# yangdongchao/RSTnet

Hardware: NVIDIA H100
Metric: codec_frames_per_s (higher is better)
Workload: dtype f32

## Files before the change

rstnet_b200/csrc/gemm_tc.cu:

```cuda
#include <cstdlib>

#include "common.cuh"
#include "tc_common.cuh"
#include "../../include/rstnet_b200.h"

namespace rstnet {
extern void count_launch();
using namespace tc;

constexpr int TC_BM = 128;
constexpr int TC_BKE = 32;
constexpr int TC_A_BYTES = TC_BM * 128;
constexpr int TC_CONSUMER_WARPS = 8;
constexpr int TC_THREADS = 32 * TC_CONSUMER_WARPS + 32;
constexpr int TC_CHUNK_STAGES = 4;

struct TcParams {
  float* C;
  float* C2;
  int act2;
  long long c_i_stride, c_o_stride, c_split_stride;
  const float* R;
  long long r_i_stride, r_o_stride, r_split_stride;
  const float* bias;
  const float* scale;
  int n_split;
  int I_out, O_out, N, Kc;
  int taps, tap_di, tap_do, o_mul, kchunks;
  int pre_act, post_act, i_tiles;
  int m_tiles, n_tiles;
  int kpair;
};

template <int BN, int PREC>
struct TcCfg {
  static constexpr bool SPLIT = PREC == 0;
  static constexpr int B_BYTES = BN * 128;
  static constexpr int STAGE_BYTES = TC_A_BYTES + B_BYTES * (SPLIT ? 2 : 1);
  static constexpr int STAGES = (200 * 1024 / STAGE_BYTES) > 8 ? 8 : (200 * 1024 / STAGE_BYTES);
  static constexpr int SMEM_BYTES = STAGES * STAGE_BYTES + 1024  + 256 ;
  static constexpr int Q_PIECES = BN / 32;
  static_assert(STAGES % 2 == 0 && 2 * Q_PIECES <= STAGES, "K-pair rings and queue");
};

__device__ __forceinline__ float tf32_rna(float x) {
  const uint32_t u = __float_as_uint(x);
  return __uint_as_float((x != x ? u | 0x00400000u : u + 0x1000u) & 0xFFFFE000u);
// ... 17 lines not shown
    for (int e = 0; e < 4; ++e) {
      const uint32_t chunk = (uint32_t)(2 * k + (e >> 1));
      float v;
      asm volatile("ld.shared.f32 %0, [%1];" : "=f"(v) : "r"(st + a_row + (e & 1) * 1024u + ((chunk ^ a_sw) << 4)));
      if (PRE_ELU) {
        const float e = __expf(v) - 1.f;
        v = v > 0.f ? v : e;
      }
      if (SPLIT) {
        const bool nonfinite = !(fabsf(v) < INFINITY);
        const float h = nonfinite ? 0.f : __uint_as_float((__float_as_uint(v) + 0x1000u) & 0xFFFFE000u);
        const float d = v - h;
        ah[k][e] = __float_as_uint(h);
        al[k][e] = (__float_as_uint(d) + (nonfinite ? 0u : 0x1000u)) & 0xFFFFE000u;
      } else {
        ah[k][e] = __float_as_uint(tf32_rna(v));
      }
    }
  }
}

template <int BN, bool SPLIT>
__device__ __forceinline__ void tc_mma_stage(float (&d0)[BN / 2], float (&d1)[BN / 2], const uint32_t (&ah)[4][4],
                                             const uint32_t (&al)[4][4], uint64_t db, uint64_t dbl, bool first) {
#pragma unroll
  for (int k = 0; k < 4; ++k) {
    const uint32_t acc_in = (first && k == 0) ? 0u : 1u;
    wgmma_tf32_rs<BN>(d0, ah[k], db + (uint64_t)(2 * k), acc_in);
    if (SPLIT) {
      wgmma_tf32_rs<BN>(d1, al[k], db + (uint64_t)(2 * k), acc_in);
      wgmma_tf32_rs<BN>(d1, ah[k], dbl + (uint64_t)(2 * k), 1u);
    }
  }
}

template <int BN, int PREC, bool PRE_ELU, bool KP>
__global__ void __launch_bounds__(TC_THREADS, 1)
gemm_tc_kernel(const __grid_constant__ CUtensorMap tmA, const __grid_constant__ CUtensorMap tmW,
               const __grid_constant__ CUtensorMap tmWlo, const TcParams p) {
  using Cfg = TcCfg<BN, PREC>;
  constexpr int S = Cfg::STAGES;
  constexpr int CH = TC_CHUNK_STAGES;
  constexpr int NR = BN / 2;
  extern __shared__ uint8_t smem_raw[];
  uint8_t* smem = smem_raw + ((1024u - (smem_u32(smem_raw) & 1023u)) & 1023u);
  uint64_t* full = reinterpret_cast<uint64_t*>(smem + S * Cfg::STAGE_BYTES);
  uint64_t* empty = full + S;
  uint64_t* qfull = empty + S;
  uint64_t* qempty = qfull + 2;
  const int warp = threadIdx.x / 32, lane = threadIdx.x % 32;
  const int total_k = p.taps * p.kchunks;
  const int total_tiles = p.m_tiles * p.n_tiles;
  const int bm = KP ? TC_BM / 2 : TC_BM;
  const int R = KP ? S / 2 : S;

  if (threadIdx.x == 0) {
    for (int s = 0; s < S; ++s) {
      mbar_init(&full[s], 1);
      mbar_init(&empty[s], KP ? TC_CONSUMER_WARPS / 2 : TC_CONSUMER_WARPS);
    }
    for (int q = 0; q < 2; ++q) {
      mbar_init(&qfull[q], 128);
      mbar_init(&qempty[q], 128);
    }
    fence_barrier_init();
  }
  __syncthreads();

  if (warp == TC_CONSUMER_WARPS) {
    if (elect_one()) {
      tma_prefetch_desc(&tmA);
      tma_prefetch_desc(&tmW);
      if (Cfg::SPLIT) tma_prefetch_desc(&tmWlo);
      int pos0 = 0, ph0 = 0, pos1 = 0, ph1 = 0;
      for (int t = blockIdx.x; t < total_tiles; t += gridDim.x) {
        const int nt = t % p.n_tiles, mt = t / p.n_tiles;
        const int i0 = (mt % p.i_tiles) * bm, ot = mt / p.i_tiles, n0 = nt * BN;
        for (int kit = 0; kit < total_k; ++kit) {
          const int w = KP ? (kit / TC_CHUNK_STAGES) & 1 : 0;
          const int pos = w ? pos1 : pos0, ph = w ? ph1 : ph0;
          const int s = w * R + pos;
          const int npos = pos + 1 == R ? 0 : pos + 1, nph = ph ^ (npos == 0);
          if (w) { pos1 = npos; ph1 = nph; } else { pos0 = npos; ph0 = nph; }
          mbar_wait(&empty[s], ph ^ 1);
          const int tap = kit / p.kchunks, kc = kit % p.kchunks;
          uint8_t* st = smem + s * Cfg::STAGE_BYTES;
          mbar_arrive_expect_tx(&full[s], Cfg::STAGE_BYTES - (TC_BM - bm) * 128);
          tma_load_3d(st, &tmA, &full[s], kc * TC_BKE, i0 + tap * p.tap_di, ot * p.o_mul + tap * p.tap_do);
          tma_load_2d(st + TC_A_BYTES, &tmW, &full[s], kit * TC_BKE, n0);
          if (Cfg::SPLIT) tma_load_2d(st + TC_A_BYTES + Cfg::B_BYTES, &tmWlo, &full[s], kit * TC_BKE, n0);
        }
      }
    }
    return;
  }

  const int wg = warp / 4, wq = warp % 4, gq = lane / 4, tq = lane % 4;
  const int r0 = (KP ? 0 : wg * 64) + wq * 16 + gq;
  const uint32_t a_row = (uint32_t)r0 * 128u + (uint32_t)tq * 4u, a_sw = (uint32_t)(r0 & 7);
  const uint32_t smem0 = smem_u32(smem);
  float acc[NR], d0[NR], d1[NR];
#pragma unroll
  for (int j = 0; j < NR; ++j) d0[j] = d1[j] = 0.f;
  const int nch = (total_k + CH - 1) / CH;
  const bool sender = KP && wg == 1;
  auto qel = [&](int q, int j) {
    return reinterpret_cast<float*>(smem + (q * Cfg::Q_PIECES + j / 16) * Cfg::STAGE_BYTES + TC_A_BYTES / 2) +
           (j % 16) * 128 + (threadIdx.x & 127);
  };
  int qn = 0;
  auto take_queued = [&]() {
    mbar_wait(&qfull[qn & 1], (qn >> 1) & 1);
#pragma unroll
    for (int j = 0; j < NR; ++j) acc[j] += *qel(qn & 1, j);
    mbar_arrive(&qempty[qn & 1]);
    ++qn;
  };
  const int base = KP ? wg * R : 0;
  int pos = 0, ph = 0;
  for (int t = blockIdx.x; t < total_tiles; t += gridDim.x) {
    const int nt = t % p.n_tiles, mt = t / p.n_tiles;
    const int i0 = (mt % p.i_tiles) * bm, ot = mt / p.i_tiles, n0 = nt * BN;
#pragma unroll
    for (int j = 0; j < NR; ++j) acc[j] = 0.f;
    for (int c = KP ? wg : 0; c < nch; c += KP ? 2 : 1) {
      const int k0 = c * CH;
      const int nst = total_k - k0 < CH ? total_k - k0 : CH;
      for (int u = 0; u < nst; ++u) {
        const int s = base + pos;
        mbar_wait(&full[s], ph);
        const uint32_t st = smem0 + (uint32_t)(s * Cfg::STAGE_BYTES);
        uint32_t ah[4][4], al[4][4];
        tc_build_a<Cfg::SPLIT, PRE_ELU>(st, a_row, a_sw, ah, al);
        const uint64_t db = gmma_desc_sw128(st + TC_A_BYTES);
        const uint64_t dbl = gmma_desc_sw128(st + TC_A_BYTES + Cfg::B_BYTES);
        wgmma_fence();
        tc_mma_stage<BN, Cfg::SPLIT>(d0, d1, ah, al, db, dbl, u == 0);
        wgmma_commit();
        wgmma_wait<0>();
        __syncwarp();
        if (lane == 0) mbar_arrive(&empty[s]);
        pos = pos + 1 == R ? 0 : pos + 1;
        ph ^= pos == 0;
      }
      fence_acc(d0);
      if (Cfg::SPLIT) fence_acc(d1);
      if (sender) {
        mbar_wait(&qempty[qn & 1], ((qn >> 1) & 1) ^ 1);
#pragma unroll
        for (int j = 0; j < NR; ++j) *qel(qn & 1, j) = Cfg::SPLIT ? d0[j] + d1[j] : d0[j];
        mbar_arrive(&qfull[qn & 1]);
        ++qn;
      } else {
        if (KP && c > 0) take_queued();
#pragma unroll
        for (int j = 0; j < NR; ++j) acc[j] += Cfg::SPLIT ? d0[j] + d1[j] : d0[j];
      }
    }
    if (KP && !sender && nch % 2 == 0) take_queued();
    if (sender) continue;
#pragma unroll
    for (int h = 0; h < 2; ++h) {
      const int i = i0 + r0 + 8 * h;
      if (i >= p.I_out) continue;
      float* crow = p.C + (long long)ot * p.c_o_stride + (long long)i * p.c_i_stride;
      float* crow2 = p.C2 ? p.C2 + (long long)ot * p.c_o_stride + (long long)i * p.c_i_stride : nullptr;
      const float* rrow = p.R ? p.R + (long long)ot * p.r_o_stride + (long long)i * p.r_i_stride : nullptr;
#pragma unroll
      for (int b = 0; b < BN / 8; ++b) {
        const int n = n0 + 8 * b + 2 * tq;
        if (n < p.N) {
          float2 v = make_float2(acc[4 * b + 2 * h], acc[4 * b + 2 * h + 1]);
          if (p.bias) {
            const float2 bb = *reinterpret_cast<const float2*>(p.bias + n);
            v.x += bb.x; v.y += bb.y;
          }
          if (p.scale) {
            const float2 ss = *reinterpret_cast<const float2*>(p.scale + n);
            v.x *= ss.x; v.y *= ss.y;
          }
          long long coff = n, roff = n;
          if (p.n_split > 0) {
            const int j = n / p.n_split, co = n % p.n_split;
            coff = (long long)j * p.c_split_stride + co;
            roff = (long long)j * p.r_split_stride + co;
          }
          if (rrow) {
            const float2 rr = *reinterpret_cast<const float2*>(rrow + roff);
            v.x += rr.x; v.y += rr.y;
          }
          if (crow2)
            *reinterpret_cast<float2*>(crow2 + coff) = make_float2(act_tc(v.x, p.act2), act_tc(v.y, p.act2));
          *reinterpret_cast<float2*>(crow + coff) = make_float2(act_tc(v.x, p.post_act), act_tc(v.y, p.post_act));
        }
      }
    }
  }
}

constexpr int RB_B_BYTES = 64 * 128;
constexpr int RB_STAGE_BYTES = TC_A_BYTES + 2 * RB_B_BYTES;
constexpr int RB_STAGES = 6;

struct RbParams {
  float* out;
  long long o_i_stride, o_o_stride;
  const float* b1;
  const float* b2;
  int I_out, i_tiles, m_tiles;
};

template <int C>
struct RbCfg {
  static constexpr int N1 = C / 2;
  static constexpr int KCH = C / 32;
  static constexpr int P1 = 3 * KCH;
  static constexpr int NS = C / 64;
  static constexpr int K2 = N1 / 32;
  static constexpr int H_BYTES = K2 * TC_A_BYTES;
  static constexpr int SMEM_BYTES = RB_STAGES * RB_STAGE_BYTES + H_BYTES + 1024  + 256 ;
  static constexpr bool ring_ok() {
    for (int j = 0; j < NS; ++j)
      for (int kc = 0; kc < KCH; ++kc)
        if ((P1 + j) % RB_STAGES == (2 * KCH + kc) % RB_STAGES) return false;
    return RB_STAGES >= KCH + NS;
  }
  static_assert(ring_ok(), "ring too small for the held residual stages");
  static_assert(K2 * 2 * RB_B_BYTES <= RB_STAGE_BYTES, "a phase-2 slice must fit one stage");
};

template <int C>
__global__ void __launch_bounds__(TC_THREADS, 1)
resblock_tc_kernel(const __grid_constant__ CUtensorMap tmY, const __grid_constant__ CUtensorMap tmW1,
                   const __grid_constant__ CUtensorMap tmW1lo, const __grid_constant__ CUtensorMap tmW2,
                   const __grid_constant__ CUtensorMap tmW2lo, const RbParams p) {
  using Cfg = RbCfg<C>;
  constexpr int S = RB_STAGES;
  constexpr int CH = TC_CHUNK_STAGES;
  constexpr int N1 = Cfg::N1, NR1 = N1 / 2, KCH = Cfg::KCH, P1 = Cfg::P1;
  extern __shared__ uint8_t smem_raw[];
  uint8_t* smem = smem_raw + ((1024u - (smem_u32(smem_raw) & 1023u)) & 1023u);
  uint8_t* hs = smem + S * RB_STAGE_BYTES;
  uint64_t* full = reinterpret_cast<uint64_t*>(hs + Cfg::H_BYTES);
  uint64_t* empty = full + S;
  const int warp = threadIdx.x / 32, lane = threadIdx.x % 32;

  if (threadIdx.x == 0) {
    for (int s = 0; s < S; ++s) {
      mbar_init(&full[s], 1);
      mbar_init(&empty[s], TC_CONSUMER_WARPS);
    }
    fence_barrier_init();
  }
  __syncthreads();

  if (warp == TC_CONSUMER_WARPS) {
    if (elect_one()) {
      tma_prefetch_desc(&tmY);
      tma_prefetch_desc(&tmW1);
      tma_prefetch_desc(&tmW1lo);
      tma_prefetch_desc(&tmW2);
      tma_prefetch_desc(&tmW2lo);
      int g = 0;
      for (int t = blockIdx.x; t < p.m_tiles; t += gridDim.x) {
        const int i0 = (t % p.i_tiles) * TC_BM, ot = t / p.i_tiles;
        for (int kit = 0; kit < P1; ++kit, ++g) {
          const int s = g % S;
          mbar_wait(&empty[s], ((g / S) & 1) ^ 1);
          const int tap = kit / KCH, kc = kit % KCH;
          uint8_t* st = smem + s * RB_STAGE_BYTES;
          mbar_arrive_expect_tx(&full[s], TC_A_BYTES + 2 * N1 * 128);
          tma_load_3d(st, &tmY, &full[s], kc * TC_BKE, i0, ot + tap);
          tma_load_2d(st + TC_A_BYTES, &tmW1, &full[s], kit * TC_BKE, 0);
          tma_load_2d(st + TC_A_BYTES + RB_B_BYTES, &tmW1lo, &full[s], kit * TC_BKE, 0);
        }
        for (int ns = 0; ns < Cfg::NS; ++ns, ++g) {
          const int s = g % S;
          mbar_wait(&empty[s], ((g / S) & 1) ^ 1);
          uint8_t* st = smem + s * RB_STAGE_BYTES;
          mbar_arrive_expect_tx(&full[s], Cfg::K2 * 2 * RB_B_BYTES);
#pragma unroll
          for (int kc = 0; kc < Cfg::K2; ++kc) {
            tma_load_2d(st + kc * 2 * RB_B_BYTES, &tmW2, &full[s], kc * TC_BKE, ns * 64);
            tma_load_2d(st + kc * 2 * RB_B_BYTES + RB_B_BYTES, &tmW2lo, &full[s], kc * TC_BKE, ns * 64);
          }
        }
      }
    }
    return;
  }

  const int wg = warp / 4, wq = warp % 4, gq = lane / 4, tq = lane % 4;
  const int r0 = wg * 64 + wq * 16 + gq;
  const uint32_t a_row = (uint32_t)r0 * 128u + (uint32_t)tq * 4u, a_sw = (uint32_t)(r0 & 7);
  const uint32_t smem0 = smem_u32(smem), hs0 = smem_u32(hs);
  int g = 0;
  for (int t = blockIdx.x; t < p.m_tiles; t += gridDim.x) {
    const int i0 = (t % p.i_tiles) * TC_BM, ot = t / p.i_tiles;
    const int g_res = g + 2 * KCH;
    {
      float acc[NR1], d0[NR1], d1[NR1];
#pragma unroll
      for (int j = 0; j < NR1; ++j) acc[j] = d0[j] = d1[j] = 0.f;
      for (int k0 = 0; k0 < P1; k0 += CH) {
        const int nst = P1 - k0 < CH ? P1 - k0 : CH;
        for (int u = 0; u < nst; ++u, ++g) {
          const int s = g % S;
          mbar_wait(&full[s], (g / S) & 1);
          const uint32_t st = smem0 + (uint32_t)(s * RB_STAGE_BYTES);
          uint32_t ah[4][4], al[4][4];
          tc_build_a<true, true>(st, a_row, a_sw, ah, al);
          wgmma_fence();
          tc_mma_stage<N1, true>(d0, d1, ah, al, gmma_desc_sw128(st + TC_A_BYTES), gmma_desc_sw128(st + TC_A_BYTES + RB_B_BYTES),
                                 u == 0);
          wgmma_commit();
          wgmma_wait<0>();
          __syncwarp();
          if (lane == 0 && k0 + u < 2 * KCH) mbar_arrive(&empty[s]);
        }
        fence_acc(d0);
        fence_acc(d1);
#pragma unroll
        for (int j = 0; j < NR1; ++j) acc[j] += d0[j] + d1[j];
      }
      named_bar_sync(1 + wg, 128);
#pragma unroll
      for (int hh = 0; hh < 2; ++hh) {
        const int r = r0 + 8 * hh;
#pragma unroll
        for (int b = 0; b < N1 / 8; ++b) {
          const int n = 8 * b + 2 * tq;
          const float2 bb = *reinterpret_cast<const float2*>(p.b1 + n);
          float2 v = make_float2(acc[4 * b + 2 * hh], acc[4 * b + 2 * hh + 1]);
          v.x += bb.x; v.y += bb.y;
          const uint32_t cc = (uint32_t)(n % 32);
          const uint32_t addr = hs0 + (uint32_t)(n / 32) * TC_A_BYTES + (uint32_t)r * 128u + (((cc >> 2) ^ (uint32_t)(r & 7)) << 4) +
                                (cc & 3u) * 4u;
          asm volatile("st.shared.v2.f32 [%0], {%1, %2};" ::"r"(addr), "f"(act_tc(v.x, ACT_ELU)), "f"(act_tc(v.y, ACT_ELU))
                       : "memory");
        }
      }
      named_bar_sync(1 + wg, 128);
    }
    for (int ns = 0; ns < Cfg::NS; ++ns, ++g) {
      const int s = g % S;
      mbar_wait(&full[s], (g / S) & 1);
      const uint32_t st = smem0 + (uint32_t)(s * RB_STAGE_BYTES);
      float acc[32], d0[32], d1[32];
#pragma unroll
      for (int j = 0; j < 32; ++j) d0[j] = d1[j] = 0.f;
#pragma unroll
      for (int kc = 0; kc < Cfg::K2; ++kc) {
        uint32_t ah[4][4], al[4][4];
        tc_build_a<true, false>(hs0 + (uint32_t)(kc * TC_A_BYTES), a_row, a_sw, ah, al);
        const uint32_t wst = st + (uint32_t)(kc * 2 * RB_B_BYTES);
        wgmma_fence();
        tc_mma_stage<64, true>(d0, d1, ah, al, gmma_desc_sw128(wst), gmma_desc_sw128(wst + RB_B_BYTES), kc == 0);
        wgmma_commit();
        wgmma_wait<0>();
      }
      __syncwarp();
      if (lane == 0) mbar_arrive(&empty[s]);
      fence_acc(d0);
      fence_acc(d1);
#pragma unroll
      for (int j = 0; j < 32; ++j) {
        acc[j] = 0.f;
        acc[j] += d0[j] + d1[j];
      }
#pragma unroll
      for (int hh = 0; hh < 2; ++hh) {
        const int r = r0 + 8 * hh;
        const int i = i0 + r;
        if (i >= p.I_out) continue;
        float* orow = p.out + (long long)ot * p.o_o_stride + (long long)i * p.o_i_stride;
#pragma unroll
        for (int b = 0; b < 8; ++b) {
          const int n = ns * 64 + 8 * b + 2 * tq;
          const float2 bb = *reinterpret_cast<const float2*>(p.b2 + n);
          float2 v = make_float2(acc[4 * b + 2 * hh], acc[4 * b + 2 * hh + 1]);
          v.x += bb.x; v.y += bb.y;
          const uint32_t cc = (uint32_t)(n % 32);
          const int rs = (g_res + n / 32) % S;
          const float2 rr = *reinterpret_cast<const float2*>(smem + rs * RB_STAGE_BYTES + r * 128 +
                                                             (((cc >> 2) ^ (uint32_t)(r & 7)) << 4) + (cc & 3u) * 4u);
          v.x += rr.x; v.y += rr.y;
          *reinterpret_cast<float2*>(orow + n) = make_float2(act_tc(v.x, ACT_ELU), act_tc(v.y, ACT_ELU));
        }
      }
      __syncwarp();
      if (lane == 0) {
        mbar_arrive(&empty[(g_res + 2 * ns) % S]);
        mbar_arrive(&empty[(g_res + 2 * ns + 1) % S]);
      }
    }
  }
}

typedef CUresult (*EncodeTiledFn)(CUtensorMap*, CUtensorMapDataType, cuuint32_t, void*, const cuuint64_t*, const cuuint64_t*,
                                  const cuuint32_t*, const cuuint32_t*, CUtensorMapInterleave, CUtensorMapSwizzle,
                                  CUtensorMapL2promotion, CUtensorMapFloatOOBfill);

static EncodeTiledFn get_encode_fn() {
  static EncodeTiledFn fn = nullptr;
  if (!fn) {
    void* p = nullptr;
    cudaDriverEntryPointQueryResult q;
    if (cudaGetDriverEntryPoint("cuTensorMapEncodeTiled", &p, cudaEnableDefault, &q) == cudaSuccess && p) fn = (EncodeTiledFn)p;
  }
  return fn;
}

}
using namespace rstnet;

struct rstnet_tc_plan {
  CUtensorMap tmA, tmW, tmWlo;
  TcParams p;
  dim3 grid;
  int bn, prec;
};

template <int BN, int PREC, bool PRE_ELU, bool KP>
static int tc_launch(const rstnet_tc_plan* pl, cudaStream_t st) {
  using Cfg = TcCfg<BN, PREC>;
  static unsigned long long attr = 0;
  smem_optin(gemm_tc_kernel<BN, PREC, PRE_ELU, KP>, Cfg::SMEM_BYTES, attr);
  gemm_tc_kernel<BN, PREC, PRE_ELU, KP><<<pl->grid, TC_THREADS, Cfg::SMEM_BYTES, st>>>(pl->tmA, pl->tmW, pl->tmWlo, pl->p);
// ... 126 lines not shown
  RSTNET_REQUIRE(d->Y && d->W1 && d->W1_lo && d->b1 && d->W2 && d->W2_lo && d->b2 && d->out, "tc_resblock_create: null pointer");
  const int Cc = d->channels;
  RSTNET_REQUIRE(Cc == 64 || Cc == 128, "tc_resblock_create: channels must be 64 or 128 (got %d)", Cc);
  RSTNET_REQUIRE(d->I_out > 0 && d->O_out > 0 && d->y_rows >= d->O_out + 2, "tc_resblock_create: bad shape");
  RSTNET_REQUIRE((uintptr_t)d->Y % 16 == 0 && (uintptr_t)d->W1 % 16 == 0 && (uintptr_t)d->W1_lo % 16 == 0 && (uintptr_t)d->W2 % 16 == 0 &&
                     (uintptr_t)d->W2_lo % 16 == 0 && (uintptr_t)d->out % 16 == 0 && (uintptr_t)d->b1 % 8 == 0 &&
                     (uintptr_t)d->b2 % 8 == 0 && d->y_i_stride % 4 == 0 && d->y_o_stride % 4 == 0 && d->out_i_stride % 4 == 0 &&
                     d->out_o_stride % 4 == 0,
                 "tc_resblock_create: 16-byte alignment required");
  RSTNET_REQUIRE(get_encode_fn() != nullptr, "tc_resblock_create: cuTensorMapEncodeTiled unavailable (no CUDA driver?)");
  rstnet_tc_resblock_plan* pl = new rstnet_tc_resblock_plan();
  pl->channels = Cc;
  int r;
  {
    cuuint64_t gdim[3] = {(cuuint64_t)Cc, (cuuint64_t)d->I_out, (cuuint64_t)d->y_rows};
    cuuint64_t gstr[2] = {(cuuint64_t)d->y_i_stride * 4, (cuuint64_t)d->y_o_stride * 4};
    cuuint32_t box[3] = {TC_BKE, TC_BM, 1};
    cuuint32_t estr[3] = {1, 1, 1};
    r = (int)get_encode_fn()(&pl->tmY, CU_TENSOR_MAP_DATA_TYPE_FLOAT32, 3, (void*)d->Y, gdim, gstr, box, estr, CU_TENSOR_MAP_INTERLEAVE_NONE,
                             CU_TENSOR_MAP_SWIZZLE_128B, CU_TENSOR_MAP_L2_PROMOTION_L2_128B, CU_TENSOR_MAP_FLOAT_OOB_FILL_NONE);
  }
  if (r == CUDA_SUCCESS) r = encode_2d(&pl->tmW1, d->W1, 3 * Cc, Cc / 2, Cc / 2);
  if (r == CUDA_SUCCESS) r = encode_2d(&pl->tmW1lo, d->W1_lo, 3 * Cc, Cc / 2, Cc / 2);
  if (r == CUDA_SUCCESS) r = encode_2d(&pl->tmW2, d->W2, Cc / 2, Cc, 64);
  if (r == CUDA_SUCCESS) r = encode_2d(&pl->tmW2lo, d->W2_lo, Cc / 2, Cc, 64);
  if (r != CUDA_SUCCESS) {
    delete pl;
    set_error("tc_resblock_create: cuTensorMapEncodeTiled failed with %d", r);
    return 3;
  }
  RbParams& p = pl->p;
  p.out = d->out; p.o_i_stride = d->out_i_stride; p.o_o_stride = d->out_o_stride;
  p.b1 = d->b1; p.b2 = d->b2;
  p.I_out = d->I_out;
  p.i_tiles = ceil_div(d->I_out, TC_BM);
  p.m_tiles = p.i_tiles * d->O_out;
  const int sms = sm_count();
  pl->grid = dim3((unsigned)(p.m_tiles < sms ? p.m_tiles : sms));
  *out = pl;
  return 0;
}

template <int Cc>
static int rb_launch(const rstnet_tc_resblock_plan* pl, cudaStream_t st) {
  constexpr int smem = RbCfg<Cc>::SMEM_BYTES;
  static unsigned long long attr = 0;
  smem_optin(resblock_tc_kernel<Cc>, smem, attr);
  resblock_tc_kernel<Cc><<<pl->grid, TC_THREADS, smem, st>>>(pl->tmY, pl->tmW1, pl->tmW1lo, pl->tmW2, pl->tmW2lo, pl->p);
  count_launch();
  return check_launch("tc_resblock");
}

extern "C" int rstnet_tc_resblock_run(const rstnet_tc_resblock_plan* pl, rstnet_stream_t stream) {
  RSTNET_REQUIRE(pl != nullptr, "tc_resblock_run: null plan");
  cudaStream_t st = (cudaStream_t)stream;
  return pl->channels == 64 ? rb_launch<64>(pl, st) : rb_launch<128>(pl, st);
}

extern "C" void rstnet_tc_resblock_destroy(rstnet_tc_resblock_plan* pl) { delete pl; }
extern "C" int rstnet_tc_gemm_grid(const rstnet_tc_plan* pl, int32_t* gx, int32_t* gy, int32_t* bn) {
  if (!pl) return 1;
  *gx = ceil_div(pl->p.I_out, TC_BM) * pl->p.O_out; *gy = pl->p.n_tiles; *bn = pl->bn;
  return 0;
}
extern "C" int rstnet_tc_gemm_kpair(const rstnet_tc_plan* pl, int32_t* on) {
  if (!pl) return 1;
  *on = pl->p.kpair;
  return 0;
}

namespace rstnet {
__global__ void tf32_split_kernel(const float* __restrict__ x, float* __restrict__ hi, float* __restrict__ lo, long long n) {
  for (long long i = (long long)blockIdx.x * blockDim.x + threadIdx.x; i < n; i += (long long)gridDim.x * blockDim.x) {
    const float v = x[i], h = tf32_rna(v);
    hi[i] = h;
    lo[i] = tf32_rna_lo(v, h);
  }
}
}

extern "C" int rstnet_tf32_split_f32(const float* x, float* hi, float* lo, int64_t n, rstnet_stream_t stream) {
// ... 9 lines not shown
```

rstnet_b200/csrc/tc_common.cuh:

```cuda
#pragma once
#include <cuda.h>
#include <cuda_runtime.h>
#include <cstdint>

namespace rstnet {
namespace tc {

__device__ __forceinline__ uint32_t smem_u32(const void* p) { return static_cast<uint32_t>(__cvta_generic_to_shared(p)); }

__device__ __forceinline__ bool elect_one() {
  uint32_t pred = 0;
  asm volatile(
      "{\n\t.reg .b32 rx;\n\t.reg .pred px;\n\t"
      "elect.sync rx|px, 0xFFFFFFFF;\n\t"
      "selp.u32 %0, 1, 0, px;\n\t}"
      : "=r"(pred));
  return pred != 0;
}

__device__ __forceinline__ void mbar_init(uint64_t* bar, uint32_t count) {
  asm volatile("mbarrier.init.shared::cta.b64 [%0], %1;" ::"r"(smem_u32(bar)), "r"(count));
}
__device__ __forceinline__ void fence_barrier_init() { asm volatile("fence.mbarrier_init.release.cluster;" ::: "memory"); }
__device__ __forceinline__ void mbar_arrive(uint64_t* bar) {
// ... 5 lines not shown
}
__device__ __forceinline__ bool mbar_try_wait(uint64_t* bar, uint32_t parity) {
  uint32_t ok;
  asm volatile(
      "{\n\t.reg .pred p;\n\t"
      "mbarrier.try_wait.parity.shared::cta.b64 p, [%1], %2;\n\t"
      "selp.u32 %0, 1, 0, p;\n\t}"
      : "=r"(ok)
      : "r"(smem_u32(bar)), "r"(parity)
      : "memory");
  return ok != 0;
}
__device__ __forceinline__ void mbar_wait(uint64_t* bar, uint32_t parity) {
  while (!mbar_try_wait(bar, parity)) {
  }
}

__device__ __forceinline__ void tma_prefetch_desc(const CUtensorMap* m) {
  asm volatile("prefetch.tensormap [%0];" ::"l"(reinterpret_cast<uint64_t>(m)) : "memory");
}
__device__ __forceinline__ void tma_load_2d(void* dst, const CUtensorMap* m, uint64_t* bar, int c0, int c1) {
  asm volatile("cp.async.bulk.tensor.2d.shared::cta.global.mbarrier::complete_tx::bytes [%0], [%1, {%3, %4}], [%2];" ::"r"(
                   smem_u32(dst)),
               "l"(reinterpret_cast<uint64_t>(m)), "r"(smem_u32(bar)), "r"(c0), "r"(c1)
               : "memory");
}
__device__ __forceinline__ void tma_load_3d(void* dst, const CUtensorMap* m, uint64_t* bar, int c0, int c1, int c2) {
  asm volatile("cp.async.bulk.tensor.3d.shared::cta.global.mbarrier::complete_tx::bytes [%0], [%1, {%3, %4, %5}], [%2];" ::"r"(
                   smem_u32(dst)),
               "l"(reinterpret_cast<uint64_t>(m)), "r"(smem_u32(bar)), "r"(c0), "r"(c1), "r"(c2)
               : "memory");
}
__device__ __forceinline__ void named_bar_sync(int id, int nthreads) { asm volatile("bar.sync %0, %1;" ::"r"(id), "r"(nthreads) : "memory"); }

__device__ __forceinline__ uint64_t gmma_desc_sw128(uint32_t saddr) {
  uint64_t d = 0;
  d |= (uint64_t)((saddr & 0x3FFFF) >> 4);
  d |= (uint64_t)1 << 16;
  d |= (uint64_t)(1024 >> 4) << 32;
  d |= (uint64_t)1 << 62;
  return d;
}
__device__ __forceinline__ void wgmma_fence() { asm volatile("wgmma.fence.sync.aligned;" ::: "memory"); }
__device__ __forceinline__ void wgmma_commit() { asm volatile("wgmma.commit_group.sync.aligned;" ::: "memory"); }
template <int N>
__device__ __forceinline__ void wgmma_wait() { asm volatile("wgmma.wait_group.sync.aligned %0;" ::"n"(N) : "memory"); }
template <int NR>
__device__ __forceinline__ void fence_acc(float (&d)[NR]) {
#pragma unroll
  for (int i = 0; i < NR; ++i) asm volatile("" : "+f"(d[i])::"memory");
}

__device__ __forceinline__ void wgmma_tf32_rs_n32(float (&d)[16], const uint32_t (&a)[4], uint64_t bdesc, uint32_t scale_d) {
  asm volatile(
      "{\n\t.reg .pred p;\n\tsetp.ne.b32 p, %21, 0;\n\t"
      "wgmma.mma_async.sync.aligned.m64n32k8.f32.tf32.tf32 "
      "{%0, %1, %2, %3, %4, %5, %6, %7, %8, %9, %10, %11, %12, %13, %14, %15}, "
      "{%16, %17, %18, %19}, %20, p, 1, 1;\n\t}"
      : "+f"(d[0]), "+f"(d[1]), "+f"(d[2]), "+f"(d[3]), "+f"(d[4]), "+f"(d[5]), "+f"(d[6]), "+f"(d[7]), "+f"(d[8]), "+f"(d[9]), "+f"(d[10]), "+f"(d[11]), "+f"(d[12]), "+f"(d[13]), "+f"(d[14]), "+f"(d[15])
      : "r"(a[0]), "r"(a[1]), "r"(a[2]), "r"(a[3]), "l"(bdesc), "r"(scale_d));
}

__device__ __forceinline__ void wgmma_tf32_rs_n64(float (&d)[32], const uint32_t (&a)[4], uint64_t bdesc, uint32_t scale_d) {
  asm volatile(
      "{\n\t.reg .pred p;\n\tsetp.ne.b32 p, %37, 0;\n\t"
      "wgmma.mma_async.sync.aligned.m64n64k8.f32.tf32.tf32 "
// ... 73 lines not shown
```

rstnet_b200/ops.py:

```python
from __future__ import annotations

import ctypes as C
import gc
from typing import Optional

import torch

from . import _lib
from ._lib import ACT_ELU, ACT_GELU, ACT_NONE, GemmRowsArgs, RowCopy, TcGemmDesc


def _stream() -> int:
    return torch.cuda.current_stream().cuda_stream


def capture(fn) -> torch.cuda.CUDAGraph:
    g = torch.cuda.CUDAGraph()
    enabled = gc.isenabled()
    gc.disable()
    try:
        with torch.cuda.graph(g):
            fn()
    finally:
        if enabled:
# ... 78 lines not shown
    def run(self):
        _lib.check(_lib.lib().rstnet_tc_gemm_run(self._h, _stream()), "tc_gemm_run")

    def __del__(self):
        h = getattr(self, "_h", None)
        if h:
            try:
                _lib.lib().rstnet_tc_gemm_destroy(h)
            except Exception:
                pass
            self._h = None


class TcResblock:

    def __init__(self, Y, y_off, y_i_stride, y_o_stride, y_rows, I_out, O_out, W1, W1_lo, b1, W2, W2_lo, b2, out, out_off,
                 out_i_stride, out_o_stride):
        _cuda(Y, W1, W1_lo, b1, W2, W2_lo, b2, out)
        Cc = W2.shape[0]
        assert tuple(W1.shape) == (Cc // 2, 3 * Cc) and tuple(W2.shape) == (Cc, Cc // 2), (W1.shape, W2.shape)
        d = _lib.TcResblockDesc()
        d.Y = Y.data_ptr() + 4 * y_off
        d.y_i_stride, d.y_o_stride = y_i_stride, y_o_stride
        d.channels, d.I_out, d.O_out, d.y_rows = Cc, I_out, O_out, y_rows
        d.W1, d.W1_lo, d.b1 = W1.data_ptr(), W1_lo.data_ptr(), b1.data_ptr()
        d.W2, d.W2_lo, d.b2 = W2.data_ptr(), W2_lo.data_ptr(), b2.data_ptr()
        d.out = out.data_ptr() + 4 * out_off
        d.out_i_stride, d.out_o_stride = out_i_stride, out_o_stride
        self._keep = (Y, W1, W1_lo, b1, W2, W2_lo, b2, out)
        self.shape = dict(C=Cc, I=I_out, O=O_out)
        n = I_out * O_out
        self.flops = 2.0 * n * (W1.numel() + W2.numel())
        self.bytes = 4.0 * (Cc * I_out * (O_out + 2) + 2 * (W1.numel() + W2.numel()) + b1.numel() + b2.numel() + n * Cc)
        self._h = C.c_void_p()
        _lib.check(_lib.lib().rstnet_tc_resblock_create(C.byref(d), C.byref(self._h)), "tc_resblock_create")

    def run(self):
        _lib.check(_lib.lib().rstnet_tc_resblock_run(self._h, _stream()), "tc_resblock_run")

    def __del__(self):
        h = getattr(self, "_h", None)
        if h:
            try:
                _lib.lib().rstnet_tc_resblock_destroy(h)
            except Exception:
                pass
            self._h = None


def conv1d_cin1(x, x_bs, x_ts, w, bias, out, out_off, out_bs, out_ts, batch, T, Cout, k, post_act=ACT_NONE, out2=None,
                out2_off=0, act2=ACT_NONE):
    _cuda(x, w, out, out2)
    _lib.check(_lib.lib().rstnet_conv1d_cin1_f32(x.data_ptr(), x_bs, x_ts, w.data_ptr(), _p(bias), out.data_ptr() + 4 * out_off,
                                                 None if out2 is None else out2.data_ptr() + 4 * out2_off, out_bs, out_ts,
                                                 batch, T, Cout, k, post_act, act2, _stream()), "conv1d_cin1")


def conv1d_cout1(x, x_bs, x_ts, w, bias, out, out_bs, batch, T, Cin, k):
    _cuda(x, w, out)
    _lib.check(_lib.lib().rstnet_conv1d_cout1_f32(x.data_ptr(), x_bs, x_ts, w.data_ptr(), _p(bias), out.data_ptr(), out_bs,
                                                  batch, T, Cin, k, _stream()), "conv1d_cout1")


def convtr1d_depthwise(x, x_bs, x_ts, w, out, out_off, out_bs, out_ts, batch, T, Cch, stride):
    _cuda(x, w, out)
    _lib.check(_lib.lib().rstnet_convtr1d_depthwise_f32(x.data_ptr(), x_bs, x_ts, w.data_ptr(), out.data_ptr() + 4 * out_off,
# ... 114 lines not shown
```

Baseline: 44550.

## Overlap consecutive WGMMA stages and add warpgroup register reallocation

Consumers now double-buffer A fragments and issue the next stage's WGMMA before waiting on the previous one (wait_group 1), releasing smem stages one step later. The producer becomes a full warpgroup that lowers its register budget via setmaxnreg while consumers raise theirs, and in KP mode two producer warps each feed their own half of the stages. The resblock second GEMM also batches all K2 MMAs before a single wait. This is meant to hide A-fragment construction and WGMMA latency behind each other. In exchange it raises register pressure from the doubled fragment arrays and adds more complex barrier release ordering.

New measurement: 45390, median of 6. 1.02x the previous value.

```diff
diff --git a/rstnet_b200/csrc/gemm_tc.cu b/rstnet_b200/csrc/gemm_tc.cu
--- a/rstnet_b200/csrc/gemm_tc.cu
+++ b/rstnet_b200/csrc/gemm_tc.cu
@@ -12,7 +12,9 @@
 constexpr int TC_BKE = 32;
 constexpr int TC_A_BYTES = TC_BM * 128;
 constexpr int TC_CONSUMER_WARPS = 8;
-constexpr int TC_THREADS = 32 * TC_CONSUMER_WARPS + 32;
+constexpr int TC_THREADS = 32 * TC_CONSUMER_WARPS + 128;
+constexpr int TC_PRODUCER_REGS = 40;
+constexpr int TC_CONSUMER_REGS = 232;
 constexpr int TC_CHUNK_STAGES = 4;
 
 struct TcParams {
@@ -96,6 +98,37 @@
       wgmma_tf32_rs<BN>(d1, ah[k], dbl + (uint64_t)(2 * k), 1u);
     }
   }
+}
+
+template <int BN, bool SPLIT, bool PRE_ELU, class Take, class Addr, class Release>
+__device__ __forceinline__ void tc_chunk(float (&d0)[BN / 2], float (&d1)[BN / 2], int nst, uint32_t a_row, uint32_t a_sw,
+                                         uint32_t b_lo, Take take, Addr addr, Release release) {
+  uint32_t ah0[4][4], al0[4][4], ah1[4][4], al1[4][4];
+  auto issue = [&](uint32_t (&ah)[4][4], uint32_t (&al)[4][4], bool first) {
+    const int tk = take();
+    const uint32_t st = addr(tk);
+    tc_build_a<SPLIT, PRE_ELU>(st, a_row, a_sw, ah, al);
+    wgmma_fence();
+    tc_mma_stage<BN, SPLIT>(d0, d1, ah, al, gmma_desc_sw128(st + TC_A_BYTES), gmma_desc_sw128(st + b_lo), first);
+    wgmma_commit();
+    return tk;
+  };
+  int held = -1, u = 0;
+  for (; u + 2 <= nst; u += 2) {
+    const int t0 = issue(ah0, al0, u == 0);
+    wgmma_wait<1>();
+    if (held >= 0) release(held);
+    held = issue(ah1, al1, false);
+    wgmma_wait<1>();
+    release(t0);
+  }
+  int tail = -1;
+  if (u < nst) tail = issue(ah0, al0, u == 0);
+  wgmma_wait<0>();
+  if (held >= 0) release(held);
+  if (tail >= 0) release(tail);
+  fence_acc(d0);
+  if (SPLIT) fence_acc(d1);
 }
 
 template <int BN, int PREC, bool PRE_ELU, bool KP>
@@ -131,34 +164,39 @@
   }
   __syncthreads();
 
-  if (warp == TC_CONSUMER_WARPS) {
-    if (elect_one()) {
+  if (warp >= TC_CONSUMER_WARPS) {
+    setmaxnreg_dec<TC_PRODUCER_REGS>();
+    const int w = warp - TC_CONSUMER_WARPS;
+    if (w < (KP ? 2 : 1) && elect_one()) {
       tma_prefetch_desc(&tmA);
       tma_prefetch_desc(&tmW);
       if (Cfg::SPLIT) tma_prefetch_desc(&tmWlo);
-      int pos0 = 0, ph0 = 0, pos1 = 0, ph1 = 0;
+      int pos = 0, ph = 0;
+      const int nch = (total_k + TC_CHUNK_STAGES - 1) / TC_CHUNK_STAGES;
       for (int t = blockIdx.x; t < total_tiles; t += gridDim.x) {
         const int nt = t % p.n_tiles, mt = t / p.n_tiles;
         const int i0 = (mt % p.i_tiles) * bm, ot = mt / p.i_tiles, n0 = nt * BN;
-        for (int kit = 0; kit < total_k; ++kit) {
-          const int w = KP ? (kit / TC_CHUNK_STAGES) & 1 : 0;
-          const int pos = w ? pos1 : pos0, ph = w ? ph1 : ph0;
-          const int s = w * R + pos;
-          const int npos = pos + 1 == R ? 0 : pos + 1, nph = ph ^ (npos == 0);
-          if (w) { pos1 = npos; ph1 = nph; } else { pos0 = npos; ph0 = nph; }
-          mbar_wait(&empty[s], ph ^ 1);
-          const int tap = kit / p.kchunks, kc = kit % p.kchunks;
-          uint8_t* st = smem + s * Cfg::STAGE_BYTES;
-          mbar_arrive_expect_tx(&full[s], Cfg::STAGE_BYTES - (TC_BM - bm) * 128);
-          tma_load_3d(st, &tmA, &full[s], kc * TC_BKE, i0 + tap * p.tap_di, ot * p.o_mul + tap * p.tap_do);
-          tma_load_2d(st + TC_A_BYTES, &tmW, &full[s], kit * TC_BKE, n0);
-          if (Cfg::SPLIT) tma_load_2d(st + TC_A_BYTES + Cfg::B_BYTES, &tmWlo, &full[s], kit * TC_BKE, n0);
+        for (int c = w; c < nch; c += KP ? 2 : 1) {
+          const int kend = (c + 1) * TC_CHUNK_STAGES < total_k ? (c + 1) * TC_CHUNK_STAGES : total_k;
+          for (int kit = c * TC_CHUNK_STAGES; kit < kend; ++kit) {
+            const int s = w * R + pos;
+            mbar_wait(&empty[s], ph ^ 1);
+            pos = pos + 1 == R ? 0 : pos + 1;
+            ph ^= pos == 0;
+            const int tap = kit / p.kchunks, kc = kit % p.kchunks;
+            uint8_t* st = smem + s * Cfg::STAGE_BYTES;
+            mbar_arrive_expect_tx(&full[s], Cfg::STAGE_BYTES - (TC_BM - bm) * 128);
+            tma_load_3d(st, &tmA, &full[s], kc * TC_BKE, i0 + tap * p.tap_di, ot * p.o_mul + tap * p.tap_do);
+            tma_load_2d(st + TC_A_BYTES, &tmW, &full[s], kit * TC_BKE, n0);
+            if (Cfg::SPLIT) tma_load_2d(st + TC_A_BYTES + Cfg::B_BYTES, &tmWlo, &full[s], kit * TC_BKE, n0);
+          }
         }
       }
     }
     return;
   }
 
+  setmaxnreg_inc<TC_CONSUMER_REGS>();
   const int wg = warp / 4, wq = warp % 4, gq = lane / 4, tq = lane % 4;
   const int r0 = (KP ? 0 : wg * 64) + wq * 16 + gq;
   const uint32_t a_row = (uint32_t)r0 * 128u + (uint32_t)tq * 4u, a_sw = (uint32_t)(r0 & 7);
@@ -182,6 +220,18 @@
   };
   const int base = KP ? wg * R : 0;
   int pos = 0, ph = 0;
+  auto take = [&]() {
+    const int s = base + pos;
+    mbar_wait(&full[s], ph);
+    pos = pos + 1 == R ? 0 : pos + 1;
+    ph ^= pos == 0;
+    return s;
+  };
+  auto addr = [&](int s) { return smem0 + (uint32_t)(s * Cfg::STAGE_BYTES); };
+  auto release = [&](int s) {
+    __syncwarp();
+    if (lane == 0) mbar_arrive(&empty[s]);
+  };
   for (int t = blockIdx.x; t < total_tiles; t += gridDim.x) {
     const int nt = t % p.n_tiles, mt = t / p.n_tiles;
     const int i0 = (mt % p.i_tiles) * bm, ot = mt / p.i_tiles, n0 = nt * BN;
@@ -190,25 +240,7 @@
     for (int c = KP ? wg : 0; c < nch; c += KP ? 2 : 1) {
       const int k0 = c * CH;
       const int nst = total_k - k0 < CH ? total_k - k0 : CH;
-      for (int u = 0; u < nst; ++u) {
-        const int s = base + pos;
-        mbar_wait(&full[s], ph);
-        const uint32_t st = smem0 + (uint32_t)(s * Cfg::STAGE_BYTES);
-        uint32_t ah[4][4], al[4][4];
-        tc_build_a<Cfg::SPLIT, PRE_ELU>(st, a_row, a_sw, ah, al);
-        const uint64_t db = gmma_desc_sw128(st + TC_A_BYTES);
-        const uint64_t dbl = gmma_desc_sw128(st + TC_A_BYTES + Cfg::B_BYTES);
-        wgmma_fence();
-        tc_mma_stage<BN, Cfg::SPLIT>(d0, d1, ah, al, db, dbl, u == 0);
-        wgmma_commit();
-        wgmma_wait<0>();
-        __syncwarp();
-        if (lane == 0) mbar_arrive(&empty[s]);
-        pos = pos + 1 == R ? 0 : pos + 1;
-        ph ^= pos == 0;
-      }
-      fence_acc(d0);
-      if (Cfg::SPLIT) fence_acc(d1);
+      tc_chunk<BN, Cfg::SPLIT, PRE_ELU>(d0, d1, nst, a_row, a_sw, TC_A_BYTES + Cfg::B_BYTES, take, addr, release);
       if (sender) {
         mbar_wait(&qempty[qn & 1], ((qn >> 1) & 1) ^ 1);
 #pragma unroll
@@ -318,8 +350,9 @@
   }
   __syncthreads();
 
-  if (warp == TC_CONSUMER_WARPS) {
-    if (elect_one()) {
+  if (warp >= TC_CONSUMER_WARPS) {
+    setmaxnreg_dec<TC_PRODUCER_REGS>();
+    if (warp == TC_CONSUMER_WARPS && elect_one()) {
       tma_prefetch_desc(&tmY);
       tma_prefetch_desc(&tmW1);
       tma_prefetch_desc(&tmW1lo);
@@ -354,36 +387,31 @@
     return;
   }
 
+  setmaxnreg_inc<TC_CONSUMER_REGS>();
   const int wg = warp / 4, wq = warp % 4, gq = lane / 4, tq = lane % 4;
   const int r0 = wg * 64 + wq * 16 + gq;
   const uint32_t a_row = (uint32_t)r0 * 128u + (uint32_t)tq * 4u, a_sw = (uint32_t)(r0 & 7);
   const uint32_t smem0 = smem_u32(smem), hs0 = smem_u32(hs);
   int g = 0;
+  auto take = [&]() {
+    mbar_wait(&full[g % S], (g / S) & 1);
+    return g++;
+  };
+  auto addr = [&](int gi) { return smem0 + (uint32_t)((gi % S) * RB_STAGE_BYTES); };
   for (int t = blockIdx.x; t < p.m_tiles; t += gridDim.x) {
     const int i0 = (t % p.i_tiles) * TC_BM, ot = t / p.i_tiles;
     const int g_res = g + 2 * KCH;
+    auto release = [&](int gi) {
+      __syncwarp();
+      if (lane == 0 && gi < g_res) mbar_arrive(&empty[gi % S]);
+    };
     {
       float acc[NR1], d0[NR1], d1[NR1];
 #pragma unroll
       for (int j = 0; j < NR1; ++j) acc[j] = d0[j] = d1[j] = 0.f;
       for (int k0 = 0; k0 < P1; k0 += CH) {
         const int nst = P1 - k0 < CH ? P1 - k0 : CH;
-        for (int u = 0; u < nst; ++u, ++g) {
-          const int s = g % S;
-          mbar_wait(&full[s], (g / S) & 1);
-          const uint32_t st = smem0 + (uint32_t)(s * RB_STAGE_BYTES);
-          uint32_t ah[4][4], al[4][4];
-          tc_build_a<true, true>(st, a_row, a_sw, ah, al);
-          wgmma_fence();
-          tc_mma_stage<N1, true>(d0, d1, ah, al, gmma_desc_sw128(st + TC_A_BYTES), gmma_desc_sw128(st + TC_A_BYTES + RB_B_BYTES),
-                                 u == 0);
-          wgmma_commit();
-          wgmma_wait<0>();
-          __syncwarp();
-          if (lane == 0 && k0 + u < 2 * KCH) mbar_arrive(&empty[s]);
-        }
-        fence_acc(d0);
-        fence_acc(d1);
+        tc_chunk<N1, true, true>(d0, d1, nst, a_row, a_sw, TC_A_BYTES + RB_B_BYTES, take, addr, release);
 #pragma unroll
         for (int j = 0; j < NR1; ++j) acc[j] += d0[j] + d1[j];
       }
@@ -413,16 +441,16 @@
       float acc[32], d0[32], d1[32];
 #pragma unroll
       for (int j = 0; j < 32; ++j) d0[j] = d1[j] = 0.f;
+      uint32_t ah[Cfg::K2][4][4], al[Cfg::K2][4][4];
 #pragma unroll
       for (int kc = 0; kc < Cfg::K2; ++kc) {
-        uint32_t ah[4][4], al[4][4];
-        tc_build_a<true, false>(hs0 + (uint32_t)(kc * TC_A_BYTES), a_row, a_sw, ah, al);
+        tc_build_a<true, false>(hs0 + (uint32_t)(kc * TC_A_BYTES), a_row, a_sw, ah[kc], al[kc]);
         const uint32_t wst = st + (uint32_t)(kc * 2 * RB_B_BYTES);
         wgmma_fence();
-        tc_mma_stage<64, true>(d0, d1, ah, al, gmma_desc_sw128(wst), gmma_desc_sw128(wst + RB_B_BYTES), kc == 0);
+        tc_mma_stage<64, true>(d0, d1, ah[kc], al[kc], gmma_desc_sw128(wst), gmma_desc_sw128(wst + RB_B_BYTES), kc == 0);
         wgmma_commit();
-        wgmma_wait<0>();
-      }
+      }
+      wgmma_wait<0>();
       __syncwarp();
       if (lane == 0) mbar_arrive(&empty[s]);
       fence_acc(d0);
diff --git a/rstnet_b200/csrc/tc_common.cuh b/rstnet_b200/csrc/tc_common.cuh
--- a/rstnet_b200/csrc/tc_common.cuh
+++ b/rstnet_b200/csrc/tc_common.cuh
@@ -61,6 +61,11 @@
                : "memory");
 }
 __device__ __forceinline__ void named_bar_sync(int id, int nthreads) { asm volatile("bar.sync %0, %1;" ::"r"(id), "r"(nthreads) : "memory"); }
+
+template <int N>
+__device__ __forceinline__ void setmaxnreg_dec() { asm volatile("setmaxnreg.dec.sync.aligned.u32 %0;" ::"n"(N)); }
+template <int N>
+__device__ __forceinline__ void setmaxnreg_inc() { asm volatile("setmaxnreg.inc.sync.aligned.u32 %0;" ::"n"(N)); }
 
 __device__ __forceinline__ uint64_t gmma_desc_sw128(uint32_t saddr) {
   uint64_t d = 0;
```

## Add window-walking resblock kernel for 64 channels with resident weights and row reuse

Applied to the files above, without the earlier changes.

Adds a new persistent resblock kernel for C=64. Each CTA walks a contiguous run of output rows and keeps a 4-slot ring of input rows, so the three conv taps reuse rows already in shared memory instead of reloading three per tile. W1 and W2 (hi/lo) are loaded once per CTA and stay resident rather than being streamed per tile. The Python side adds an L2 byte-count estimate. This cuts redundant global/L2 traffic, at the cost of serializing the wgmma waits per stage and possibly unbalanced run boundaries.

Result: no change. 44760 before, 44830 after, median of 6 (+0.2%).

```diff
diff --git a/rstnet_b200/csrc/gemm_tc.cu b/rstnet_b200/csrc/gemm_tc.cu
--- a/rstnet_b200/csrc/gemm_tc.cu
+++ b/rstnet_b200/csrc/gemm_tc.cu
@@ -271,7 +271,7 @@
   long long o_i_stride, o_o_stride;
   const float* b1;
   const float* b2;
-  int I_out, i_tiles, m_tiles;
+  int I_out, O_out, i_tiles, m_tiles;
 };
 
 template <int C>
@@ -458,6 +458,198 @@
         mbar_arrive(&empty[(g_res + 2 * ns + 1) % S]);
       }
     }
+  }
+}
+
+namespace rbw {
+constexpr int C = 64, N1 = 32, KCH = 2, P1 = 3 * KCH;
+constexpr int ROW_BYTES = KCH * TC_A_BYTES;
+constexpr int SLOTS = 4;
+constexpr int W1_STAGE = N1 * 128;
+constexpr int W2_BYTES = C * 128;
+constexpr int WIN = 0;
+constexpr int W1HI = WIN + SLOTS * ROW_BYTES;
+constexpr int W1LO = W1HI + P1 * W1_STAGE;
+constexpr int W2HI = W1LO + P1 * W1_STAGE;
+constexpr int W2LO = W2HI + W2_BYTES;
+constexpr int HS = W2LO + W2_BYTES;
+constexpr int BARS = HS + TC_A_BYTES;
+constexpr int W_BYTES = 2 * P1 * W1_STAGE + 2 * W2_BYTES;
+constexpr int SMEM_BYTES = BARS + 1024  + 256 ;
+static_assert(SMEM_BYTES <= 227 * 1024, "window, weights and h must fit one SM");
+
+struct Run {
+  int it, o0, o1;
+};
+__device__ __forceinline__ Run run_at(long long q, long long q_end, int O_out) {
+  Run r;
+  r.it = (int)(q / O_out);
+  r.o0 = (int)(q % O_out);
+  const long long left = q_end - q;
+  r.o1 = left < (long long)(O_out - r.o0) ? r.o0 + (int)left : O_out;
+  return r;
+}
+}
+
+__global__ void __launch_bounds__(TC_THREADS, 1)
+resblock_walk_kernel(const __grid_constant__ CUtensorMap tmY, const __grid_constant__ CUtensorMap tmW1,
+                     const __grid_constant__ CUtensorMap tmW1lo, const __grid_constant__ CUtensorMap tmW2,
+                     const __grid_constant__ CUtensorMap tmW2lo, const RbParams p) {
+  using namespace rbw;
+  constexpr int CH = TC_CHUNK_STAGES;
+  constexpr int NR1 = N1 / 2;
+  extern __shared__ uint8_t smem_raw[];
+  uint8_t* smem = smem_raw + ((1024u - (smem_u32(smem_raw) & 1023u)) & 1023u);
+  uint64_t* full = reinterpret_cast<uint64_t*>(smem + BARS);
+  uint64_t* empty = full + SLOTS;
+  uint64_t* wfull = empty + SLOTS;
+  const int warp = threadIdx.x / 32, lane = threadIdx.x % 32;
+  const long long items = (long long)p.m_tiles;
+  const long long q_begin = items * blockIdx.x / gridDim.x, q_end = items * (blockIdx.x + 1) / gridDim.x;
+
+  if (threadIdx.x == 0) {
+    for (int s = 0; s < SLOTS; ++s) {
+      mbar_init(&full[s], 1);
+      mbar_init(&empty[s], TC_CONSUMER_WARPS);
+    }
+    mbar_init(wfull, 1);
+    fence_barrier_init();
+  }
+  __syncthreads();
+
+  if (warp == TC_CONSUMER_WARPS) {
+    if (elect_one()) {
+      tma_prefetch_desc(&tmY);
+      tma_prefetch_desc(&tmW1);
+      tma_prefetch_desc(&tmW1lo);
+      tma_prefetch_desc(&tmW2);
+      tma_prefetch_desc(&tmW2lo);
+      mbar_arrive_expect_tx(wfull, W_BYTES);
+      for (int kit = 0; kit < P1; ++kit) {
+        tma_load_2d(smem + W1HI + kit * W1_STAGE, &tmW1, wfull, kit * TC_BKE, 0);
+        tma_load_2d(smem + W1LO + kit * W1_STAGE, &tmW1lo, wfull, kit * TC_BKE, 0);
+      }
+      tma_load_2d(smem + W2HI, &tmW2, wfull, 0, 0);
+      tma_load_2d(smem + W2LO, &tmW2lo, wfull, 0, 0);
+      int g = 0;
+      for (long long q = q_begin; q < q_end;) {
+        const Run r = run_at(q, q_end, p.O_out);
+        q += r.o1 - r.o0;
+        for (int row = r.o0; row < r.o1 + 2; ++row, ++g) {
+          const int s = g % SLOTS;
+          mbar_wait(&empty[s], ((g / SLOTS) & 1) ^ 1);
+          uint8_t* st = smem + WIN + s * ROW_BYTES;
+          mbar_arrive_expect_tx(&full[s], ROW_BYTES);
+#pragma unroll
+          for (int kc = 0; kc < KCH; ++kc) tma_load_3d(st + kc * TC_A_BYTES, &tmY, &full[s], kc * TC_BKE, r.it * TC_BM, row);
+        }
+      }
+    }
+    return;
+  }
+
+  const int wg = warp / 4, wq = warp % 4, gq = lane / 4, tq = lane % 4;
+  const int r0 = wg * 64 + wq * 16 + gq;
+  const uint32_t a_row = (uint32_t)r0 * 128u + (uint32_t)tq * 4u, a_sw = (uint32_t)(r0 & 7);
+  const uint32_t smem0 = smem_u32(smem), hs0 = smem0 + HS;
+  mbar_wait(wfull, 0);
+  int g = 0;
+  for (long long q = q_begin; q < q_end;) {
+    const Run run = run_at(q, q_end, p.O_out);
+    q += run.o1 - run.o0;
+    const int i0 = run.it * TC_BM;
+    for (int ot = run.o0; ot < run.o1; ++ot) {
+      const int g0 = g + (ot - run.o0);
+      {
+        float acc[NR1], d0[NR1], d1[NR1];
+#pragma unroll
+        for (int j = 0; j < NR1; ++j) acc[j] = d0[j] = d1[j] = 0.f;
+        for (int k0 = 0; k0 < P1; k0 += CH) {
+          const int nst = P1 - k0 < CH ? P1 - k0 : CH;
+          for (int u = 0; u < nst; ++u) {
+            const int kit = k0 + u, tap = kit / KCH, kc = kit % KCH;
+            const int gr = g0 + tap, s = gr % SLOTS;
+            mbar_wait(&full[s], (gr / SLOTS) & 1);
+            const uint32_t st = smem0 + (uint32_t)(WIN + s * ROW_BYTES + kc * TC_A_BYTES);
+            uint32_t ah[4][4], al[4][4];
+            tc_build_a<true, true>(st, a_row, a_sw, ah, al);
+            wgmma_fence();
+            tc_mma_stage<N1, true>(d0, d1, ah, al, gmma_desc_sw128(smem0 + W1HI + kit * W1_STAGE),
+                                   gmma_desc_sw128(smem0 + W1LO + kit * W1_STAGE), u == 0);
+            wgmma_commit();
+            wgmma_wait<0>();
+            __syncwarp();
+            if (lane == 0 && kit == KCH - 1) mbar_arrive(&empty[s]);
+          }
+          fence_acc(d0);
+          fence_acc(d1);
+#pragma unroll
+          for (int j = 0; j < NR1; ++j) acc[j] += d0[j] + d1[j];
+        }
+        named_bar_sync(1 + wg, 128);
+#pragma unroll
+        for (int hh = 0; hh < 2; ++hh) {
+          const int r = r0 + 8 * hh;
+#pragma unroll
+          for (int b = 0; b < N1 / 8; ++b) {
+            const int n = 8 * b + 2 * tq;
+            const float2 bb = *reinterpret_cast<const float2*>(p.b1 + n);
+            float2 v = make_float2(acc[4 * b + 2 * hh], acc[4 * b + 2 * hh + 1]);
+            v.x += bb.x; v.y += bb.y;
+            const uint32_t cc = (uint32_t)(n % 32);
+            const uint32_t addr = hs0 + (uint32_t)r * 128u + (((cc >> 2) ^ (uint32_t)(r & 7)) << 4) + (cc & 3u) * 4u;
+            asm volatile("st.shared.v2.f32 [%0], {%1, %2};" ::"r"(addr), "f"(act_tc(v.x, ACT_ELU)), "f"(act_tc(v.y, ACT_ELU))
+                         : "memory");
+          }
+        }
+        named_bar_sync(1 + wg, 128);
+      }
+      float acc[32], d0[32], d1[32];
+#pragma unroll
+      for (int j = 0; j < 32; ++j) d0[j] = d1[j] = 0.f;
+      {
+        uint32_t ah[4][4], al[4][4];
+        tc_build_a<true, false>(hs0, a_row, a_sw, ah, al);
+        wgmma_fence();
+        tc_mma_stage<64, true>(d0, d1, ah, al, gmma_desc_sw128(smem0 + W2HI), gmma_desc_sw128(smem0 + W2LO), true);
+        wgmma_commit();
+        wgmma_wait<0>();
+      }
+      fence_acc(d0);
+      fence_acc(d1);
+#pragma unroll
+      for (int j = 0; j < 32; ++j) {
+        acc[j] = 0.f;
+        acc[j] += d0[j] + d1[j];
+      }
+      const uint8_t* yres = smem + WIN + ((g0 + 2) % SLOTS) * ROW_BYTES;
+#pragma unroll
+      for (int hh = 0; hh < 2; ++hh) {
+        const int r = r0 + 8 * hh;
+        const int i = i0 + r;
+        if (i >= p.I_out) continue;
+        float* orow = p.out + (long long)ot * p.o_o_stride + (long long)i * p.o_i_stride;
+#pragma unroll
+        for (int b = 0; b < 8; ++b) {
+          const int n = 8 * b + 2 * tq;
+          const float2 bb = *reinterpret_cast<const float2*>(p.b2 + n);
+          float2 v = make_float2(acc[4 * b + 2 * hh], acc[4 * b + 2 * hh + 1]);
+          v.x += bb.x; v.y += bb.y;
+          const uint32_t cc = (uint32_t)(n % 32);
+          const float2 rr = *reinterpret_cast<const float2*>(yres + (n / 32) * TC_A_BYTES + r * 128 +
+                                                             (((cc >> 2) ^ (uint32_t)(r & 7)) << 4) + (cc & 3u) * 4u);
+          v.x += rr.x; v.y += rr.y;
+          *reinterpret_cast<float2*>(orow + n) = make_float2(act_tc(v.x, ACT_ELU), act_tc(v.y, ACT_ELU));
+        }
+      }
+    }
+    const int n_out = run.o1 - run.o0;
+    __syncwarp();
+    if (lane == 0) {
+      mbar_arrive(&empty[(g + n_out) % SLOTS]);
+      mbar_arrive(&empty[(g + n_out + 1) % SLOTS]);
+    }
+    g += n_out + 2;
   }
 }
 
@@ -650,7 +842,7 @@
   RbParams& p = pl->p;
   p.out = d->out; p.o_i_stride = d->out_i_stride; p.o_o_stride = d->out_o_stride;
   p.b1 = d->b1; p.b2 = d->b2;
-  p.I_out = d->I_out;
+  p.I_out = d->I_out; p.O_out = d->O_out;
   p.i_tiles = ceil_div(d->I_out, TC_BM);
   p.m_tiles = p.i_tiles * d->O_out;
   const int sms = sm_count();
@@ -661,10 +853,15 @@
 
 template <int Cc>
 static int rb_launch(const rstnet_tc_resblock_plan* pl, cudaStream_t st) {
-  constexpr int smem = RbCfg<Cc>::SMEM_BYTES;
+  auto kernel = resblock_walk_kernel;
+  int smem = rbw::SMEM_BYTES;
+  if constexpr (Cc != 64) {
+    kernel = resblock_tc_kernel<Cc>;
+    smem = RbCfg<Cc>::SMEM_BYTES;
+  }
   static unsigned long long attr = 0;
-  smem_optin(resblock_tc_kernel<Cc>, smem, attr);
-  resblock_tc_kernel<Cc><<<pl->grid, TC_THREADS, smem, st>>>(pl->tmY, pl->tmW1, pl->tmW1lo, pl->tmW2, pl->tmW2lo, pl->p);
+  smem_optin(kernel, smem, attr);
+  kernel<<<pl->grid, TC_THREADS, smem, st>>>(pl->tmY, pl->tmW1, pl->tmW1lo, pl->tmW2, pl->tmW2lo, pl->p);
   count_launch();
   return check_launch("tc_resblock");
 }
diff --git a/rstnet_b200/ops.py b/rstnet_b200/ops.py
--- a/rstnet_b200/ops.py
+++ b/rstnet_b200/ops.py
@@ -134,6 +134,16 @@
         n = I_out * O_out
         self.flops = 2.0 * n * (W1.numel() + W2.numel())
         self.bytes = 4.0 * (Cc * I_out * (O_out + 2) + 2 * (W1.numel() + W2.numel()) + b1.numel() + b2.numel() + n * Cc)
+        groups = -(-I_out // 128)
+        self.tiles = groups * O_out
+        row = 4 * 128 * Cc
+        w = 8 * (W1.numel() + W2.numel())
+        if Cc == 64:
+            ctas = min(self.tiles, torch.cuda.get_device_properties(Y.device).multi_processor_count)
+            runs = sum((self.tiles * (b + 1) // ctas - 1) // O_out - (self.tiles * b // ctas) // O_out + 1 for b in range(ctas))
+            self.l2_bytes = row * (self.tiles + 2 * runs) + w * ctas
+        else:
+            self.l2_bytes = (3 * row + w) * self.tiles
         self._h = C.c_void_p()
         _lib.check(_lib.lib().rstnet_tc_resblock_create(C.byref(d), C.byref(self._h)), "tc_resblock_create")
 
```
